# archinetai/audio-diffusion-pytorch

Hardware: NVIDIA H100
Metric: audio-seconds/sec (2ch, 2^18 len) VSampler 50-step (higher is better)
Workload: dtype bf16

## Files before the change

audio_diffusion_pytorch_b200/_build.py:

```python
import os
import subprocess
import sys
from concurrent.futures import ThreadPoolExecutor

PKG_DIR = os.path.dirname(os.path.abspath(__file__))
CSRC = os.path.join(PKG_DIR, "csrc")
LIB_PATH = os.path.join(PKG_DIR, "libadp_b200.so")
SOURCES = ["common.cu", "conv_gemm.cu", "rowwise.cu", "stem.cu", "mid_conv.cu", "attention.cu", "attention_bwd.cu", "backward.cu", "wgrad.cu", "stem_bwd.cu", "frontend.cu", "stft_loss.cu", "verify_f32.cu", "verify_f32_bwd.cu"]
NVCC_FLAGS = [
    "-gencode", "arch=compute_90a,code=sm_90a", "-lineinfo", "-O3", "-std=c++17",
    "-Xcompiler", "-fPIC", "--expt-relaxed-constexpr", "-Xptxas", "-v",
]


def _nvcc() -> str:
    for cand in (os.environ.get("NVCC"), "/usr/local/cuda/bin/nvcc", "nvcc"):
        if cand and (os.path.isabs(cand) and os.path.exists(cand) or not os.path.isabs(cand)):
            return cand
    raise RuntimeError("nvcc not found")


def _sources():
    return [s for s in SOURCES if os.path.exists(os.path.join(CSRC, s))]


def needs_build() -> bool:
    if not os.path.exists(LIB_PATH):
        return True
    lib_m = os.path.getmtime(LIB_PATH)
    deps = [os.path.join(CSRC, f) for f in os.listdir(CSRC)]
    deps.append(os.path.join(os.path.dirname(PKG_DIR), "include", "adp_b200.h"))
    return any(os.path.getmtime(d) > lib_m for d in deps if os.path.exists(d))


def build(force: bool = False, verbose: bool = False) -> str:
    if not force and not needs_build():
        return LIB_PATH
    nvcc = _nvcc()
    objdir = os.path.join(PKG_DIR, "build")
    os.makedirs(objdir, exist_ok=True)

    def compile_one(src: str) -> str:
        obj = os.path.join(objdir, src.replace(".cu", ".o"))
        cmd = [nvcc, *NVCC_FLAGS, "-c", os.path.join(CSRC, src), "-o", obj]
        r = subprocess.run(cmd, capture_output=True, text=True)
        log = os.path.join(objdir, src + ".log")
        with open(log, "w") as fh:
            fh.write(" ".join(cmd) + "\n" + r.stdout + r.stderr)
        if r.returncode != 0:
            raise RuntimeError(f"nvcc failed for {src}:\n{r.stdout}\n{r.stderr}")
        if verbose:
            print(r.stderr, file=sys.stderr)
        return obj

    with ThreadPoolExecutor(max_workers=8) as ex:
        objs = list(ex.map(compile_one, _sources()))
    cmd = [nvcc, "-shared", "-o", LIB_PATH, *objs, "-gencode", "arch=compute_90a,code=sm_90a"]
    r = subprocess.run(cmd, capture_output=True, text=True)
    if r.returncode != 0:
        raise RuntimeError(f"link failed:\n{r.stdout}\n{r.stderr}")
    return LIB_PATH


if __name__ == "__main__":
    print(build(force="--force" in sys.argv, verbose="-v" in sys.argv))
```

audio_diffusion_pytorch_b200/csrc/conv_gemm.cu:

```cuda
#include "common.cuh"
#include "ptx.cuh"

namespace adp {

int g_debug[8] = {0, 0, 0, 0, 0, 0, 0, 0};

constexpr int kMaxStages = 8;
constexpr int kMaxGroups = 8;
constexpr int kSmemPerSM = 228 * 1024;
constexpr int kSmemPerBlock = 227 * 1024;

struct Gemm2Params {
  __nv_bfloat16* out;
  const __nv_bfloat16* residual;
  const float* bias;
  const float* gate;
  double* stats;
  int B, T, tiles_per_batch, c_in, ldo;
  int n_pad, n_valid;
  int ntaps, tap_off0, up_factor;
  int groups, group_size, group_shift;
  int out_fp32, ld_gate;
  int n_tiles_n, total_tiles, tiles_per_cta;
  int a_rows;
  int kc;
  int k_stages;
  int n_stages;
  int a_sub_bytes, w_sub_bytes, stage_bytes, max_taps;
  int early_w;
  const double* gn_stats;
  const float* gn_gamma;
  const float* gn_beta;
  float gn_eps;
  int gn_groups;
};

struct TileInfo {
  int b, t0, n0, phase, ch0, ntaps, min_off;
};

template <int BM>
__device__ __forceinline__ TileInfo tile_info(const Gemm2Params& p, int tile, int BN) {
  TileInfo ti;
  const int m_tile = tile / p.n_tiles_n;
  const int n_tile = tile - m_tile * p.n_tiles_n;
  ti.b = m_tile / p.tiles_per_batch;
  ti.t0 = (m_tile - ti.b * p.tiles_per_batch) * BM;
  ti.n0 = n_tile * BN;
  ti.phase = ti.n0 / p.n_pad;
  ti.ch0 = ti.n0 - ti.phase * p.n_pad;
  if (p.up_factor > 1) {
    if (ti.phase == 0) { ti.ntaps = 2; ti.min_off = -1; }
    else if (ti.phase == p.up_factor - 1) { ti.ntaps = 2; ti.min_off = 0; }
    else { ti.ntaps = 1; ti.min_off = 0; }
  } else {
    ti.ntaps = p.ntaps;
    ti.min_off = p.tap_off0;
  }
  return ti;
}

__device__ __forceinline__ float silu_tanh(float z) {
  float t;
  asm("tanh.approx.f32 %0, %1;" : "=f"(t) : "f"(0.5f * z));
  const float hz = 0.5f * z;
  return fmaf(hz, t, hz);
}

struct WarpStats {
  int cur_g = -1;
  float s = 0.f, q = 0.f;
  template <int NW>
  __device__ __forceinline__ void flush(float (*slots)[NW], int w, int lane) {
    const float ws = warp_sum(s), wq = warp_sum(q);
    if (lane == 0 && cur_g >= 0) { slots[2 * cur_g][w] += ws; slots[2 * cur_g + 1][w] += wq; }
    s = 0.f; q = 0.f;
  }
  template <int NW>
  __device__ __forceinline__ void add(float v, int g, float (*slots)[NW], int w, int lane) {
    if (g != cur_g) { flush(slots, w, lane); cur_g = g; }
    s += v; q += v * v;
  }
};

struct NarrowStats {
  int ch0 = -1;
  float s[4] = {0.f, 0.f, 0.f, 0.f}, q[4] = {0.f, 0.f, 0.f, 0.f};
  __device__ __forceinline__ void add(int k, float v) { s[k] += v; q[k] += v * v; }
  template <int NW>
  __device__ __forceinline__ void flush(float (*slots)[NW], int w, int lane, int shift, int groups) {
    if (ch0 >= 0) {
#pragma unroll
      for (int k = 0; k < 4; ++k) {
        float a = s[k], b = q[k];
#pragma unroll
        for (int o = 4; o < 32; o <<= 1) {
          a += __shfl_xor_sync(0xffffffffu, a, o);
          b += __shfl_xor_sync(0xffffffffu, b, o);
        }
        if (shift == 2) {
          a += __shfl_xor_sync(0xffffffffu, a, 1);
          b += __shfl_xor_sync(0xffffffffu, b, 1);
        }
        const int col = shift == 0 ? ch0 + 2 * lane + k : ch0 + 8 * k + 2 * (lane & 3);
        const int g = col >> shift;
        if (lane < 4 && (shift != 2 || !(lane & 1)) && (shift != 0 || k < 2) && g < groups) {
          slots[2 * g][w] += a;
          slots[2 * g + 1][w] += b;
        }
        s[k] = 0.f; q[k] = 0.f;
      }
    }
    ch0 = -1;
  }
};

template <int BM> constexpr int gemm_threads() { return 2 * BM + 32; }

template <int BM, int BN, int SW, bool XF, bool NARROW>
__global__ void __launch_bounds__(gemm_threads<BM>(), BM == 256 ? 1 : (BN <= 32 ? 3 : (BN <= 64 ? 2 : 1)))
conv_gemm2_kernel(const __grid_constant__ CUtensorMap tmA, const __grid_constant__ CUtensorMap tmW,
                  const Gemm2Params p) {
  static_assert(!NARROW || (BN <= 64 && !XF), "narrow statistics registers: BN <= 64 without XF");
  static_assert(BM == 128 || (BM == 256 && BN == 64 && !XF && !NARROW),
                "256-row tiles: BN = 64, without the A transform or the narrow statistics");
  constexpr int BK = SW / 2;
  constexpr int NACC = BN / 2;
  constexpr int kConsumers = 2 * BM;
  constexpr int kConsumerWarps = BM / 16;
  constexpr uint32_t kWTapBytes = BN * SW;
  extern __shared__ uint8_t smem_raw[];
  __shared__ uint64_t full_bar[kMaxStages], empty_bar[kMaxStages];
  __shared__ float s_part[2 * kMaxGroups][kConsumerWarps];
  __shared__ __align__(16) float s_coef[XF ? 2 * 1024 : 4];

  pdl_launch_dependents();
  const int warp = warp_id_uniform();
  const int lane = threadIdx.x & 31;
  const uint32_t raw = smem_u32(smem_raw);
  uint8_t* ring = smem_raw + ((1024u - (raw & 1023u)) & 1023u);

  const int tile_begin = blockIdx.x * p.tiles_per_cta;
  int tile_end = tile_begin + p.tiles_per_cta;
  if (tile_end > p.total_tiles) tile_end = p.total_tiles;

  if (threadIdx.x < 2 * kMaxGroups * kConsumerWarps) (&s_part[0][0])[threadIdx.x] = 0.f;
  if (warp == kConsumerWarps && lane == 0) {
    for (int s = 0; s < p.n_stages; ++s) { mbar_init(&full_bar[s], 1); mbar_init(&empty_bar[s], kConsumerWarps); }
    fence_mbar_init();
    tma_prefetch_desc(&tmA);
    tma_prefetch_desc(&tmW);
  }
  __syncthreads();
  if (warp == kConsumerWarps) {
    const uint32_t a_bytes = static_cast<uint32_t>(BM / 128) * p.a_rows * SW;
    const int total_it = (tile_end - tile_begin) * p.k_stages;
    int early = 0;
    if (p.early_w) {
      early = total_it < p.n_stages ? total_it : p.n_stages;
      if (elect_one()) {
        int tile = tile_begin, ks = 0;
        for (int it = 0; it < early; ++it) {
          const TileInfo ti = tile_info<BM>(p, tile, BN);
          uint8_t* st = ring + it * p.stage_bytes;
          mbar_arrive_expect_tx(&full_bar[it], static_cast<uint32_t>(p.kc) * (a_bytes + ti.ntaps * kWTapBytes));
          for (int c = 0; c < p.kc; ++c) {
            const int k0 = (ks * p.kc + c) * BK;
            uint8_t* wdst = st + p.kc * p.a_sub_bytes + c * p.max_taps * p.w_sub_bytes;
            for (int tap = 0; tap < ti.ntaps; ++tap)
              tma_load_2d(wdst + tap * p.w_sub_bytes, &tmW, &full_bar[it], tap * p.c_in + k0, ti.n0);
          }
          if (++ks == p.k_stages) { ks = 0; ++tile; }
        }
      }
      __syncwarp();
    }
    pdl_wait();
    int s = 0, it = 0;
    uint32_t ph = 0;
    for (int tile = tile_begin; tile < tile_end; ++tile) {
      const TileInfo ti = tile_info<BM>(p, tile, BN);
      const uint32_t tx = static_cast<uint32_t>(p.kc) * (a_bytes + ti.ntaps * kWTapBytes);
      for (int ks = 0; ks < p.k_stages; ++ks, ++it) {
        const bool armed = it < early;
        if (!armed) mbar_wait(&empty_bar[s], ph ^ 1);
        uint8_t* st = ring + s * p.stage_bytes;
        if (elect_one()) {
          if (!armed) mbar_arrive_expect_tx(&full_bar[s], tx);
          for (int c = 0; c < p.kc; ++c) {
            const int k0 = (ks * p.kc + c) * BK;
            tma_load_3d(st + c * p.a_sub_bytes, &tmA, &full_bar[s], k0, ti.t0 + ti.min_off, ti.b);
            if constexpr (BM == 256)
              tma_load_3d(st + c * p.a_sub_bytes + 128 * SW, &tmA, &full_bar[s], k0, ti.t0 + ti.min_off + 128, ti.b);
            if (armed) continue;
            uint8_t* wdst = st + p.kc * p.a_sub_bytes + c * p.max_taps * p.w_sub_bytes;
            for (int tap = 0; tap < ti.ntaps; ++tap)
              tma_load_2d(wdst + tap * p.w_sub_bytes, &tmW, &full_bar[s], tap * p.c_in + k0, ti.n0);
          }
        }
        __syncwarp();
        if (++s == p.n_stages) { s = 0; ph ^= 1; }
      }
    }
    return;
  }

  pdl_wait();
  const int tid = threadIdx.x;
  const int wg = tid >> 7;
  const int r0 = wg * 64 + (warp & 3) * 16 + (lane >> 2);
  const int cq = 2 * (lane & 3);
  const bool do_stats = p.stats != nullptr;
  const bool narrow = NARROW && p.group_shift >= 0 && p.group_shift < 3;
  WarpStats acc_st;
  NarrowStats nar_st;
  int cur_b = -1, coef_b = -1;

  auto publish_stats = [&](int b_done) {
    acc_st.flush(s_part, warp, lane);
    acc_st.cur_g = -1;
    if (narrow) nar_st.flush(s_part, warp, lane, p.group_shift, p.groups);
    named_bar_sync(1, kConsumers);
    if (tid < 2 * p.groups) {
      float tot = 0.f;
#pragma unroll
      for (int w = 0; w < kConsumerWarps; ++w) { tot += s_part[tid][w]; s_part[tid][w] = 0.f; }
      if (tot != 0.f) atomicAdd(p.stats + static_cast<size_t>(b_done) * 2 * p.groups + tid, static_cast<double>(tot));
    }
    named_bar_sync(1, kConsumers);
  };

  const uint64_t desc0 = gmma_desc_kmajor<SW>(smem_u32(ring));
  const uint32_t stage_u = static_cast<uint32_t>(p.stage_bytes) >> 4;
  const uint32_t a_sub_u = static_cast<uint32_t>(p.a_sub_bytes) >> 4;
  const uint32_t w_sub_u = static_cast<uint32_t>(p.w_sub_bytes) >> 4;
  const uint32_t w_base_u = static_cast<uint32_t>(p.kc) * a_sub_u;
  const uint32_t wg_row_u = static_cast<uint32_t>(wg * 64 * SW) >> 4;
  int s = 0;
  uint32_t ph = 0;
  for (int tile = tile_begin; tile < tile_end; ++tile) {
    const TileInfo ti = tile_info<BM>(p, tile, BN);
    if constexpr (XF) {
      if (ti.b != coef_b) {
        named_bar_sync(1, kConsumers);
        const int gsz = p.c_in / p.gn_groups;
        const double inv_n = 1.0 / (static_cast<double>(gsz) * p.T);
        for (int ch = tid; ch < p.c_in; ch += kConsumers) {
          const int g = ch / gsz;
          const double mean = p.gn_stats[(static_cast<size_t>(ti.b) * p.gn_groups + g) * 2] * inv_n;
          const float var = fmaxf(static_cast<float>(
              p.gn_stats[(static_cast<size_t>(ti.b) * p.gn_groups + g) * 2 + 1] * inv_n - mean * mean), 0.f);
          const float ga = __ldg(p.gn_gamma + ch) * rsqrtf(var + p.gn_eps);
          s_coef[2 * ch] = ga;
          s_coef[2 * ch + 1] = __ldg(p.gn_beta + ch) - static_cast<float>(mean) * ga;
        }
        named_bar_sync(1, kConsumers);
        coef_b = ti.b;
      }
    }
    float acc[NACC];
    uint32_t accumulate = 0;
    int prev_s = -1;
    for (int ks = 0; ks < p.k_stages; ++ks) {
      mbar_wait(&full_bar[s], ph);
      if constexpr (XF) {
        constexpr int CPR = SW / 16;
        constexpr int CPT = CPR / 2 > 0 ? CPR / 2 : 1;
        uint8_t* st = ring + s * p.stage_bytes;
        for (int c = 0; c < p.kc; ++c) {
          uint8_t* sub = st + c * p.a_sub_bytes;
          const float* cf = s_coef + (ks * p.kc + c) * BK * 2;
          for (int rr = tid >> 1; rr < p.a_rows; rr += kConsumers / 2) {
            const int t = ti.t0 + ti.min_off + rr;
            if (t < 0 || t >= p.T) continue;
            const uint32_t row_off = static_cast<uint32_t>(rr) * SW;
            const int swz = (row_off >> 7) & (CPR - 1);
#pragma unroll
            for (int q = 0; q < CPT; ++q) {
              const int pc = (CPR >= 2) ? (tid & 1) * CPT + q : 0;
              if (CPR < 2 && (tid & 1)) continue;
              const int lc = pc ^ swz;
              uint4* ptr = reinterpret_cast<uint4*>(sub + row_off + pc * 16);
              const uint4 u = *ptr;
              const float4* c4 = reinterpret_cast<const float4*>(cf + lc * 16);
              const float4 k0 = c4[0], k1 = c4[1], k2 = c4[2], k3 = c4[3];
              const float2 f0 = unpack_bf16(u.x), f1 = unpack_bf16(u.y);
              const float2 f2 = unpack_bf16(u.z), f3 = unpack_bf16(u.w);
              uint4 o;
              o.x = pack_bf16(silu_tanh(f0.x * k0.x + k0.y), silu_tanh(f0.y * k0.z + k0.w));
              o.y = pack_bf16(silu_tanh(f1.x * k1.x + k1.y), silu_tanh(f1.y * k1.z + k1.w));
              o.z = pack_bf16(silu_tanh(f2.x * k2.x + k2.y), silu_tanh(f2.y * k2.z + k2.w));
              o.w = pack_bf16(silu_tanh(f3.x * k3.x + k3.y), silu_tanh(f3.y * k3.z + k3.w));
              *ptr = o;
            }
          }
        }
        fence_proxy_async_smem();
        named_bar_sync(1, kConsumers);
      }
      wgmma_fence();
      const uint64_t sdesc = desc0 + static_cast<uint64_t>(s * stage_u);
      for (int c = 0; c < p.kc; ++c) {
        const uint64_t adesc = sdesc + c * a_sub_u + wg_row_u;
        const uint64_t wdesc = sdesc + w_base_u + c * p.max_taps * w_sub_u;
        for (int tap = 0; tap < ti.ntaps; ++tap) {
#pragma unroll
          for (int kk = 0; kk < BK / 16; ++kk) {
            Wgmma<BN>::template ss<0, 0>(acc, adesc + ((tap * SW + kk * 32) >> 4),
                                         wdesc + tap * w_sub_u + ((kk * 32) >> 4), accumulate);
            accumulate = 1;
          }
        }
      }
      wgmma_commit();
      wgmma_wait<1>();
      if (prev_s >= 0) {
        __syncwarp();
        if (lane == 0) mbar_arrive(&empty_bar[prev_s]);
      }
      prev_s = s;
      if (++s == p.n_stages) { s = 0; ph ^= 1; }
    }
    wgmma_wait<0>();
    acc_fence(acc);
    __syncwarp();
    if (lane == 0) mbar_arrive(&empty_bar[prev_s]);

    if (do_stats && ti.b != cur_b) {
      if (cur_b >= 0) publish_stats(cur_b);
      cur_b = ti.b;
    }
    if (narrow && ti.ch0 != nar_st.ch0) {
      nar_st.flush(s_part, warp, lane, p.group_shift, p.groups);
      nar_st.ch0 = ti.ch0;
    }
    const int t_lo = ti.t0 + r0, t_hi = t_lo + 8;
    const bool ok_lo = t_lo < p.T, ok_hi = t_hi < p.T;
    const size_t col_off = static_cast<size_t>(ti.phase) * p.n_valid;
    const size_t off_lo = (static_cast<size_t>(ti.b) * p.T + (ok_lo ? t_lo : 0)) * p.ldo + col_off;
    const size_t off_hi = (static_cast<size_t>(ti.b) * p.T + (ok_hi ? t_hi : 0)) * p.ldo + col_off;
    const float* gate_row = p.gate ? p.gate + static_cast<size_t>(ti.b) * p.ld_gate : nullptr;
#pragma unroll
    for (int jb = 0; jb < BN / 8; ++jb) {
      if (ti.ch0 + jb * 8 >= p.n_valid) break;
      const int ch = ti.ch0 + jb * 8 + cq;
      const float2 bb = p.bias ? make_float2(__ldg(p.bias + ch), __ldg(p.bias + ch + 1)) : make_float2(0.f, 0.f);
      const float2 gg = gate_row ? make_float2(__ldg(gate_row + ch), __ldg(gate_row + ch + 1)) : make_float2(1.f, 1.f);
      float v[4];
      v[0] = (acc[4 * jb + 0] + bb.x) * gg.x; v[1] = (acc[4 * jb + 1] + bb.y) * gg.y;
      v[2] = (acc[4 * jb + 2] + bb.x) * gg.x; v[3] = (acc[4 * jb + 3] + bb.y) * gg.y;
      if (p.out_fp32) {
        float* o = reinterpret_cast<float*>(p.out);
        if (ok_lo) *reinterpret_cast<float2*>(o + off_lo + ch) = make_float2(v[0], v[1]);
        if (ok_hi) *reinterpret_cast<float2*>(o + off_hi + ch) = make_float2(v[2], v[3]);
        continue;
      }
      if (p.residual) {
        if (ok_lo) {
          const float2 r = unpack_bf16(__ldg(reinterpret_cast<const unsigned int*>(p.residual + off_lo + ch)));
          v[0] += r.x; v[1] += r.y;
        }
        if (ok_hi) {
          const float2 r = unpack_bf16(__ldg(reinterpret_cast<const unsigned int*>(p.residual + off_hi + ch)));
          v[2] += r.x; v[3] += r.y;
        }
      }
      const uint32_t o_lo = pack_bf16(v[0], v[1]), o_hi = pack_bf16(v[2], v[3]);
      if (ok_lo) *reinterpret_cast<uint32_t*>(p.out + off_lo + ch) = o_lo;
      if (ok_hi) *reinterpret_cast<uint32_t*>(p.out + off_hi + ch) = o_hi;
      if (do_stats) {
        const float2 q_lo = ok_lo ? unpack_bf16(o_lo) : make_float2(0.f, 0.f);
        const float2 q_hi = ok_hi ? unpack_bf16(o_hi) : make_float2(0.f, 0.f);
        if (p.group_shift >= 3) {
          const int g = (ti.ch0 + jb * 8) >> p.group_shift;
          acc_st.add(q_lo.x, g, s_part, warp, lane); acc_st.add(q_lo.y, g, s_part, warp, lane);
          acc_st.add(q_hi.x, g, s_part, warp, lane); acc_st.add(q_hi.y, g, s_part, warp, lane);
        } else if (narrow) {
          if (p.group_shift == 0) {
            nar_st.add(0, q_lo.x); nar_st.add(0, q_hi.x);
            nar_st.add(1, q_lo.y); nar_st.add(1, q_hi.y);
          } else if (jb < 4) {
            nar_st.add(jb, q_lo.x); nar_st.add(jb, q_lo.y);
            nar_st.add(jb, q_hi.x); nar_st.add(jb, q_hi.y);
          }
        } else {
          float cs[2] = {q_lo.x + q_hi.x, q_lo.y + q_hi.y};
          float cs2[2] = {q_lo.x * q_lo.x + q_hi.x * q_hi.x, q_lo.y * q_lo.y + q_hi.y * q_hi.y};
#pragma unroll
          for (int e = 0; e < 2; ++e)
#pragma unroll
            for (int o = 4; o < 32; o <<= 1) {
              cs[e] += __shfl_xor_sync(0xffffffffu, cs[e], o);
              cs2[e] += __shfl_xor_sync(0xffffffffu, cs2[e], o);
            }
#pragma unroll
          for (int i = 0; i < 8; ++i) {
            const float v = __shfl_sync(0xffffffffu, cs[i & 1], i >> 1);
            const float v2 = __shfl_sync(0xffffffffu, cs2[i & 1], i >> 1);
            const int g = (ti.ch0 + jb * 8 + i) / p.group_size;
            if (lane == 0) { s_part[2 * g][warp] += v; s_part[2 * g + 1][warp] += v2; }
          }
        }
      }
    }
  }
  if (do_stats && cur_b >= 0) publish_stats(cur_b);
}

template <int BM, int BN, int SW, bool XF, bool NARROW>
static int launch_gemm2(const adp_conv_gemm_args& a, cudaStream_t stream) {
  constexpr int BK = SW / 2;
  constexpr int kThreads = gemm_threads<BM>();
  auto kernel = conv_gemm2_kernel<BM, BN, SW, XF, NARROW>;
  const int tiles_per_batch = (a.T + BM - 1) / BM;
  const bool up = a.up_factor > 1;
  const int max_taps = up ? 2 : a.ntaps;
  const int span = up ? 1 : a.ntaps - 1;
  const int a_rows = 128 + span;
  const int k_chunks = a.c_in / BK;

  Gemm2Params p;
  p.a_sub_bytes = ((BM + span) * SW + 1023) / 1024 * 1024;
  p.w_sub_bytes = (BN * SW + 1023) / 1024 * 1024;
  p.max_taps = max_taps;
  const int chunk_bytes = p.a_sub_bytes + max_taps * p.w_sub_bytes;

  const int w_iters = k_chunks * max_taps;
  int occ = 1;
  if (BM == 256) occ = 1;
  else if (BN <= 64 && w_iters <= 8) occ = 3;
  else if (BN <= 128 && w_iters <= 12) occ = 2;
  if (XF && occ > (BN <= 64 ? 2 : 1)) occ = BN <= 64 ? 2 : 1;
  if (g_debug[3] > 0) occ = g_debug[3];
  static int static_smem = -1;
  if (static_smem < 0) {
    cudaFuncAttributes fa;
    ADP_CUDA(cudaFuncGetAttributes(&fa, kernel));
    static_smem = static_cast<int>(fa.sharedSizeBytes);
  }
  auto budget_of = [&](int o) {
    int per_cta = kSmemPerSM / o - 1024;
    if (per_cta > kSmemPerBlock) per_cta = kSmemPerBlock;
    return per_cta - static_smem - 1024;
  };
  while (occ > 1 && budget_of(occ) < 2 * chunk_bytes) --occ;
  const int budget = budget_of(occ);
  int kc = 1;
  while (kc * 2 <= 4 && k_chunks % (kc * 2) == 0 && kc * max_taps * (BK / 16) < 8 &&
         2 * (kc * 2) * chunk_bytes <= budget)
    kc *= 2;
  if (g_debug[5] > 0 && k_chunks % g_debug[5] == 0) kc = g_debug[5];
  p.kc = kc;
  p.k_stages = k_chunks / kc;
  p.stage_bytes = kc * chunk_bytes;
  int n_stages = budget / p.stage_bytes;
  if (n_stages > kMaxStages) n_stages = kMaxStages;
  if (n_stages < 2)
    return set_error("adp_conv_gemm: stage of %d bytes does not fit (BN=%d)", p.stage_bytes, BN);
  p.n_stages = n_stages;
  const size_t smem = static_cast<size_t>(n_stages) * p.stage_bytes + 1024;

  CUtensorMap tmA, tmW;
  {
    const uint64_t dims[3] = {(uint64_t)a.c_in, (uint64_t)a.T, (uint64_t)a.B};
    const uint64_t strides[2] = {(uint64_t)a.lda * 2, (uint64_t)a.T * a.lda * 2};
    const uint32_t box[3] = {(uint32_t)BK, (uint32_t)a_rows, 1};
    if (int e = make_tmap_bf16(&tmA, a.a, 3, dims, strides, box, SW)) return e;
  }
  {
    const uint64_t dims[2] = {(uint64_t)a.k_total, (uint64_t)a.phases * a.n_pad};
    const uint64_t strides[1] = {(uint64_t)a.k_total * 2};
    const uint32_t box[2] = {(uint32_t)BK, (uint32_t)BN};
    if (int e = make_tmap_bf16(&tmW, a.w, 2, dims, strides, box, SW)) return e;
  }

  static SmemAttrCache smem_cache;
  ADP_CUDA(ensure_dyn_smem(kernel, smem, smem_cache));
  int occ_hw = 1;
  if (cudaOccupancyMaxActiveBlocksPerMultiprocessor(&occ_hw, kernel, kThreads, smem) != cudaSuccess ||
      occ_hw < 1)
    occ_hw = 1;
  if (occ > occ_hw) occ = occ_hw;

  p.out = static_cast<__nv_bfloat16*>(a.out);
  p.residual = static_cast<const __nv_bfloat16*>(a.residual);
  p.bias = a.bias;
  p.gate = a.gate;
  p.stats = a.stats;
  p.B = a.B;
  p.T = a.T;
  p.tiles_per_batch = tiles_per_batch;
  p.c_in = a.c_in;
  p.ldo = a.ldo;
  p.n_pad = a.n_pad;
  p.n_valid = a.n_valid;
  p.ntaps = a.ntaps;
  p.tap_off0 = a.tap_off[0];
  p.up_factor = a.up_factor;
  p.groups = a.stats ? a.groups : 0;
  p.group_size = a.stats ? a.n_valid / a.groups : 1;
  p.group_shift = -1;
  for (int sft = 0; sft < 16; ++sft)
    if ((1 << sft) == p.group_size) p.group_shift = sft;
  p.out_fp32 = a.out_fp32;
  p.ld_gate = a.ld_gate > 0 ? a.ld_gate : a.n_valid;
  p.n_tiles_n = a.phases * a.n_pad / BN;
  p.total_tiles = a.B * tiles_per_batch * p.n_tiles_n;
  p.a_rows = a_rows;
  p.early_w = g_debug[2];
  p.gn_stats = a.gn_stats;
  p.gn_gamma = a.gn_gamma;
  p.gn_beta = a.gn_beta;
  p.gn_eps = a.gn_eps;
  p.gn_groups = a.gn_groups > 0 ? a.gn_groups : 1;

  const int slots = occ * num_sms();
  int grid = p.total_tiles < slots ? p.total_tiles : slots;
  p.tiles_per_cta = (p.total_tiles + grid - 1) / grid;
  grid = (p.total_tiles + p.tiles_per_cta - 1) / p.tiles_per_cta;
  ADP_CUDA(launch_k(kernel, dim3(grid), dim3(kThreads), smem, stream, tmA, tmW, p));
  ADP_LAUNCH_CHECK();
  return 0;
}

static bool needs_narrow(const adp_conv_gemm_args& a) {
  const int group_size = a.stats ? a.n_valid / a.groups : 0;
  return group_size == 1 || group_size == 2 || group_size == 4 || g_debug[7] != 0;
}

template <int SW>
static int dispatch_bn2(const adp_conv_gemm_args& a, int bn, cudaStream_t s) {
  if (a.gn_stats) {
    switch (bn) {
      case 16: return launch_gemm2<128, 16, SW, true, false>(a, s);
      case 32: return launch_gemm2<128, 32, SW, true, false>(a, s);
      case 64: return launch_gemm2<128, 64, SW, true, false>(a, s);
      case 128: return launch_gemm2<128, 128, SW, true, false>(a, s);
      case 256: return launch_gemm2<128, 256, SW, true, false>(a, s);
    }
  }
  const bool narrow = needs_narrow(a);
  switch (bn) {
    case 16: return narrow ? launch_gemm2<128, 16, SW, false, true>(a, s) : launch_gemm2<128, 16, SW, false, false>(a, s);
    case 32: return narrow ? launch_gemm2<128, 32, SW, false, true>(a, s) : launch_gemm2<128, 32, SW, false, false>(a, s);
    case 64: return narrow ? launch_gemm2<128, 64, SW, false, true>(a, s) : launch_gemm2<128, 64, SW, false, false>(a, s);
    case 128: return launch_gemm2<128, 128, SW, false, false>(a, s);
    case 256: return launch_gemm2<128, 256, SW, false, false>(a, s);
  }
  return set_error("adp_conv_gemm: unsupported N tile %d", bn);
}

static bool has_256_rows(const adp_conv_gemm_args& a) {
  return a.n_pad % 64 == 0 && a.c_in % 64 == 0 && !a.gn_stats && !needs_narrow(a) && a.T >= 256;
}

}

namespace adp { extern int g_mid_threads; }

extern "C" int adp_debug_set(int key, int value) {
  if (key == 8) {
    if (value != 128 && value != 256) return adp::set_error("adp_debug_set: key 8 takes 128 or 256");
    adp::g_mid_threads = value;
    return 0;
  }
  if (key < 0 || key >= 8) return adp::set_error("adp_debug_set: bad key %d", key);
  if (key == 4 && value != 0 && value != 128 && value != 256)
    return adp::set_error("adp_debug_set: key 4 takes 0, 128 or 256");
  adp::g_debug[key] = value;
  if (key == 6) adp::g_pdl = value;
  return 0;
}

extern "C" int adp_conv_gemm(const adp_conv_gemm_args* args, adp_stream_t stream) {
  using namespace adp;
  ADP_CHECK(args != nullptr, "adp_conv_gemm: null args");
  const adp_conv_gemm_args& a = *args;
  ADP_CHECK(a.a && a.w && a.out, "adp_conv_gemm: null a/w/out");
  ADP_CHECK(a.B > 0 && a.T > 0, "adp_conv_gemm: bad B=%d T=%d", a.B, a.T);
  ADP_CHECK(a.c_in >= 16 && a.c_in % 16 == 0, "adp_conv_gemm: c_in=%d must be a multiple of 16",
            a.c_in);
  ADP_CHECK(a.lda % 8 == 0 && a.ldo % 8 == 0 && a.k_total % 8 == 0 && a.lda >= a.c_in,
            "adp_conv_gemm: pitches lda=%d ldo=%d k_total=%d must be multiples of 8", a.lda, a.ldo,
            a.k_total);
  ADP_CHECK(a.n_valid > 0 && a.n_valid % 8 == 0 && a.n_valid <= a.n_pad && a.n_pad % 16 == 0,
            "adp_conv_gemm: n_valid=%d n_pad=%d", a.n_valid, a.n_pad);
  ADP_CHECK(a.phases >= 1, "adp_conv_gemm: phases=%d", a.phases);
  ADP_CHECK(a.ld_gate % 4 == 0, "adp_conv_gemm: ld_gate=%d must be a multiple of 4", a.ld_gate);
  if (a.up_factor > 1) {
    ADP_CHECK(a.phases == a.up_factor, "adp_conv_gemm: phases (%d) != up_factor (%d)", a.phases,
              a.up_factor);
    ADP_CHECK(a.k_total >= 2 * a.c_in, "adp_conv_gemm: upsample weights need 2 tap slots");
  } else {
    ADP_CHECK(a.ntaps >= 1 && a.ntaps <= 3 && a.phases == 1, "adp_conv_gemm: ntaps=%d phases=%d",
              a.ntaps, a.phases);
    ADP_CHECK(a.k_total >= a.ntaps * a.c_in, "adp_conv_gemm: k_total too small");
    for (int i = 1; i < a.ntaps; ++i)
      ADP_CHECK(a.tap_off[i] == a.tap_off[i - 1] + 1,
                "adp_conv_gemm: tap offsets must be consecutive and ascending");
  }
  if (a.out_fp32) {
    ADP_CHECK(!a.residual && !a.stats, "adp_conv_gemm: out_fp32 excludes residual/stats");
  }
  if (a.gn_stats) {
    ADP_CHECK(a.c_in <= 1024, "adp_conv_gemm: fused GroupNorm supports c_in <= 1024");
    ADP_CHECK(a.gn_gamma && a.gn_beta && a.gn_groups > 0 && a.c_in % a.gn_groups == 0 && a.lda == a.c_in,
              "adp_conv_gemm: fused GroupNorm needs gamma/beta, groups | c_in and a dense input");
  }
  if (a.stats) {
    ADP_CHECK(a.groups > 0 && a.groups <= kMaxGroups && a.n_valid % a.groups == 0,
              "adp_conv_gemm: groups=%d n_valid=%d (fused statistics handle <= %d groups)",
              a.groups, a.n_valid, kMaxGroups);
  }
  int bn = a.block_n;
  if (bn == 0) {
    const long m_tiles = (long)a.B * ((a.T + 127) / 128);
    const int k_per_tile = (a.up_factor > 1 ? 2 : a.ntaps) * a.c_in;
    const int widest = !a.gn_stats && k_per_tile <= 1024 ? 64 : 128;
    bn = 16;
    for (int cand = widest; cand >= 16; cand >>= 1) {
      if (a.n_pad % cand) continue;
      const long tiles = m_tiles * (a.phases * a.n_pad / cand);
      if (tiles >= 96 || cand <= 64) { bn = cand; break; }
    }
  }
  bool rows256 = false;
  if (g_debug[4] == 256) {
    ADP_CHECK(has_256_rows(a) && (a.block_n == 0 || a.block_n == 64),
              "adp_conv_gemm: no 256-row tile for block_n=%d c_in=%d T=%d", a.block_n, a.c_in, a.T);
    rows256 = true;
  } else if (a.block_n == 0 && g_debug[4] != 128) {
    rows256 = bn == 128 && has_256_rows(a);
  }
  ADP_CHECK(a.n_pad % bn == 0, "adp_conv_gemm: N tile %d does not divide n_pad %d", bn, a.n_pad);
  cudaStream_t s = as_stream(stream);
  if (rows256) return launch_gemm2<256, 64, 128, false, false>(a, s);
  if (a.c_in % 64 == 0) return dispatch_bn2<128>(a, bn, s);
  if (a.c_in % 32 == 0) return dispatch_bn2<64>(a, bn, s);
  return dispatch_bn2<32>(a, bn, s);
}
```

Before: 173.5.

## Add specialized thin-channel GEMM kernel for small conv and upsample shapes

```diff
diff --git a/audio_diffusion_pytorch_b200/_build.py b/audio_diffusion_pytorch_b200/_build.py
--- a/audio_diffusion_pytorch_b200/_build.py
+++ b/audio_diffusion_pytorch_b200/_build.py
@@ -6,7 +6,7 @@
 PKG_DIR = os.path.dirname(os.path.abspath(__file__))
 CSRC = os.path.join(PKG_DIR, "csrc")
 LIB_PATH = os.path.join(PKG_DIR, "libadp_b200.so")
-SOURCES = ["common.cu", "conv_gemm.cu", "rowwise.cu", "stem.cu", "mid_conv.cu", "attention.cu", "attention_bwd.cu", "backward.cu", "wgrad.cu", "stem_bwd.cu", "frontend.cu", "stft_loss.cu", "verify_f32.cu", "verify_f32_bwd.cu"]
+SOURCES = ["common.cu", "conv_gemm.cu", "rowwise.cu", "stem.cu", "mid_conv.cu", "thin_gemm.cu", "attention.cu", "attention_bwd.cu", "backward.cu", "wgrad.cu", "stem_bwd.cu", "frontend.cu", "stft_loss.cu", "verify_f32.cu", "verify_f32_bwd.cu"]
 NVCC_FLAGS = [
     "-gencode", "arch=compute_90a,code=sm_90a", "-lineinfo", "-O3", "-std=c++17",
     "-Xcompiler", "-fPIC", "--expt-relaxed-constexpr", "-Xptxas", "-v",
diff --git a/audio_diffusion_pytorch_b200/csrc/conv_gemm.cu b/audio_diffusion_pytorch_b200/csrc/conv_gemm.cu
--- a/audio_diffusion_pytorch_b200/csrc/conv_gemm.cu
+++ b/audio_diffusion_pytorch_b200/csrc/conv_gemm.cu
@@ -556,12 +556,22 @@
 
 }
 
-namespace adp { extern int g_mid_threads; }
+namespace adp {
+extern int g_mid_threads;
+bool thin_gemm_fits(const adp_conv_gemm_args& a);
+int thin_gemm(const adp_conv_gemm_args& a, cudaStream_t stream);
+int g_thin_off = 0;
+}
 
 extern "C" int adp_debug_set(int key, int value) {
   if (key == 8) {
     if (value != 128 && value != 256) return adp::set_error("adp_debug_set: key 8 takes 128 or 256");
     adp::g_mid_threads = value;
+    return 0;
+  }
+  if (key == 9) {
+    if (value != 0 && value != 1) return adp::set_error("adp_debug_set: key 9 takes 0 or 1");
+    adp::g_thin_off = value;
     return 0;
   }
   if (key < 0 || key >= 8) return adp::set_error("adp_debug_set: bad key %d", key);
@@ -612,6 +622,7 @@
               "adp_conv_gemm: groups=%d n_valid=%d (fused statistics handle <= %d groups)",
               a.groups, a.n_valid, kMaxGroups);
   }
+  if (!g_thin_off && thin_gemm_fits(a)) return thin_gemm(a, as_stream(stream));
   int bn = a.block_n;
   if (bn == 0) {
     const long m_tiles = (long)a.B * ((a.T + 127) / 128);
diff --git a/audio_diffusion_pytorch_b200/csrc/thin_gemm.cu b/audio_diffusion_pytorch_b200/csrc/thin_gemm.cu
--- /dev/null
+++ b/audio_diffusion_pytorch_b200/csrc/thin_gemm.cu
@@ -0,0 +1,262 @@
+#include "common.cuh"
+#include "ptx.cuh"
+
+namespace adp {
+
+extern int g_debug[8];
+
+__device__ __forceinline__ void cp_async16(uint32_t dst, const void* src, uint32_t src_bytes) {
+  asm volatile("cp.async.cg.shared.global [%0], [%1], 16, %2;" ::"r"(dst), "l"(src), "r"(src_bytes) : "memory");
+}
+__device__ __forceinline__ void cp_async_commit() { asm volatile("cp.async.commit_group;" ::: "memory"); }
+__device__ __forceinline__ void cp_async_wait_1() { asm volatile("cp.async.wait_group 1;" ::: "memory"); }
+
+template <int CIN, int NV, int F, int TB>
+struct ThinCfg {
+  static constexpr int NTH = 2 * TB;
+  static constexpr int HALO = F > 1 ? 1 : 0;
+  static constexpr int AR = TB + 2 * HALO;
+  static constexpr int RS = CIN * 2 + 16;
+  static constexpr int KP = (F > 1 ? 2 : 1) * CIN;
+  static constexpr int WS = KP * 2 + 16;
+  static constexpr int NT = NV / 8;
+  static constexpr int WOUT = F * NV;
+  static constexpr int OS = WOUT + 4;
+  static constexpr int LPR = WOUT / 8;
+  static constexpr int RPP = NTH / LPR;
+  static constexpr int EP = (TB + RPP - 1) / RPP;
+  static constexpr int A_BYTES = AR * RS;
+  static constexpr int O_FLOATS = TB * OS > NTH * 16 ? TB * OS : NTH * 16;
+  static constexpr int W_BYTES = F * NV * WS;
+  static constexpr int SMEM = 2 * A_BYTES + O_FLOATS * 4 + W_BYTES;
+  static_assert(NV % 8 == 0 && CIN % 16 == 0 && TB % 16 == 0 && RPP >= 1, "thin GEMM shape");
+};
+
+template <int CIN, int NV, int F, int TB>
+__global__ void __launch_bounds__(2 * TB, TB == 128 ? 3 : 2) thin_gemm_kernel(const adp_conv_gemm_args a, int early_w) {
+  using Cfg = ThinCfg<CIN, NV, F, TB>;
+  constexpr int NTH = Cfg::NTH, HALO = Cfg::HALO, AR = Cfg::AR, RS = Cfg::RS, KP = Cfg::KP;
+  constexpr int WS = Cfg::WS, NT = Cfg::NT, WOUT = Cfg::WOUT, OS = Cfg::OS, LPR = Cfg::LPR;
+  constexpr int RPP = Cfg::RPP, EP = Cfg::EP;
+  extern __shared__ __align__(128) uint8_t smem[];
+  uint8_t* s_a = smem;
+  float* s_o = reinterpret_cast<float*>(smem + 2 * Cfg::A_BYTES);
+  uint8_t* s_w = smem + 2 * Cfg::A_BYTES + Cfg::O_FLOATS * 4;
+  __shared__ float s_ch[2 * WOUT];
+
+  pdl_launch_dependents();
+  const int b = blockIdx.y;
+  const int tid = threadIdx.x, warp = tid >> 5, lane = tid & 31;
+  const int T = a.T;
+  const int n_tiles = (T + TB - 1) / TB;
+  const __nv_bfloat16* ab = static_cast<const __nv_bfloat16*>(a.a) + static_cast<size_t>(b) * T * a.lda;
+  const size_t orow = static_cast<size_t>(b) * T;
+  const uint32_t a_base = smem_u32(s_a), w_base = smem_u32(s_w);
+
+  auto load_w = [&]() {
+    constexpr int VPR = KP / 8;
+    const __nv_bfloat16* w = static_cast<const __nv_bfloat16*>(a.w);
+    for (int i = tid; i < F * NV * VPR; i += NTH) {
+      const int row = i / VPR, v = i - row * VPR;
+      const int p = row / NV, n = row - p * NV;
+      if (F > 1 && p > 0 && p < F - 1 && v >= CIN / 8) continue;
+      cp_async16(w_base + row * WS + v * 16, w + static_cast<size_t>(p * a.n_pad + n) * a.k_total + v * 8, 16u);
+    }
+  };
+  if (early_w) load_w();
+  pdl_wait();
+  if (!early_w) load_w();
+
+  auto load_a = [&](int tile, int buf) {
+    constexpr int CH = CIN / 8;
+    const int t_first = tile * TB - HALO;
+    for (int i = tid; i < AR * CH; i += NTH) {
+      const int r = i / CH, c = i - r * CH;
+      const int t = t_first + r;
+      const bool ok = t >= 0 && t < T;
+      const __nv_bfloat16* src = ok ? ab + static_cast<size_t>(t) * a.lda + c * 8 : ab;
+      cp_async16(a_base + buf * Cfg::A_BYTES + r * RS + c * 16, src, ok ? 16u : 0u);
+    }
+  };
+
+  int tile = blockIdx.x;
+  if (tile < n_tiles) load_a(tile, 0);
+  cp_async_commit();
+
+  const int el = tid % LPR, row0 = tid / LPR;
+  const bool e_on = row0 < RPP;
+  const int c0 = (el * 8) % NV;
+  float bb[8], gg[8];
+  {
+    const float* gate_row = a.gate ? a.gate + static_cast<size_t>(b) * (a.ld_gate > 0 ? a.ld_gate : a.n_valid) : nullptr;
+#pragma unroll
+    for (int j = 0; j < 8; ++j) {
+      bb[j] = a.bias ? __ldg(a.bias + c0 + j) : 0.f;
+      gg[j] = gate_row ? __ldg(gate_row + c0 + j) : 1.f;
+    }
+  }
+  const bool has_res = a.residual != nullptr;
+  const __nv_bfloat16* res = static_cast<const __nv_bfloat16*>(a.residual);
+  __nv_bfloat16* out = static_cast<__nv_bfloat16*>(a.out);
+  float st_s[8], st_q[8];
+#pragma unroll
+  for (int j = 0; j < 8; ++j) { st_s[j] = 0.f; st_q[j] = 0.f; }
+
+  for (int it = 0; tile < n_tiles; tile += gridDim.x, ++it) {
+    const int buf = it & 1;
+    const int t0 = tile * TB;
+    if (tile + gridDim.x < n_tiles) load_a(tile + gridDim.x, buf ^ 1);
+    cp_async_commit();
+    uint4 rv[EP];
+#pragma unroll
+    for (int i = 0; i < EP; ++i) {
+      const int t = t0 + row0 + i * RPP;
+      rv[i] = make_uint4(0, 0, 0, 0);
+      if (has_res && e_on && row0 + i * RPP < TB && t < T)
+        rv[i] = __ldg(reinterpret_cast<const uint4*>(res + (orow + t) * a.ldo + el * 8));
+    }
+    cp_async_wait_1();
+    __syncthreads();
+
+    const uint32_t ab_s = a_base + buf * Cfg::A_BYTES;
+    const int g = lane >> 2, q = lane & 3;
+#pragma unroll
+    for (int p = 0; p < F; ++p) {
+      const int ntap = (F > 1 && (p == 0 || p == F - 1)) ? 2 : 1;
+      const int off = (F > 1 && p == 0) ? -1 : 0;
+      float acc[NT][4];
+#pragma unroll
+      for (int j = 0; j < NT; ++j) acc[j][0] = acc[j][1] = acc[j][2] = acc[j][3] = 0.f;
+#pragma unroll
+      for (int tap = 0; tap < 2; ++tap) {
+        if (tap >= ntap) break;
+#pragma unroll
+        for (int c16 = 0; c16 < CIN / 16; ++c16) {
+          uint32_t af[4];
+          ldmatrix_x4(ab_s + static_cast<uint32_t>(warp * 16 + (lane & 7) + ((lane >> 3) & 1) * 8 + HALO + off + tap) * RS +
+                      (c16 * 16 + ((lane >> 4) & 1) * 8) * 2, af);
+          const uint32_t wk = w_base + static_cast<uint32_t>(p * NV) * WS + (tap * CIN + c16 * 16) * 2;
+#pragma unroll
+          for (int np = 0; np < NT / 2; ++np) {
+            uint32_t bf[4];
+            ldmatrix_x4(wk + static_cast<uint32_t>(np * 16 + (lane & 7) + ((lane >> 4) & 1) * 8) * WS +
+                        ((lane >> 3) & 1) * 16, bf);
+            mma_16816(acc[2 * np], af, bf[0], bf[1]);
+            mma_16816(acc[2 * np + 1], af, bf[2], bf[3]);
+          }
+          if constexpr (NT % 2 == 1) {
+            uint32_t bf[2];
+            ldmatrix_x2(wk + static_cast<uint32_t>((NT - 1) * 8 + (lane & 7)) * WS + ((lane >> 3) & 1) * 16, bf);
+            mma_16816(acc[NT - 1], af, bf[0], bf[1]);
+          }
+        }
+      }
+      const int r = warp * 16 + g;
+#pragma unroll
+      for (int j = 0; j < NT; ++j) {
+        *reinterpret_cast<float2*>(s_o + r * OS + p * NV + 8 * j + 2 * q) = make_float2(acc[j][0], acc[j][1]);
+        *reinterpret_cast<float2*>(s_o + (r + 8) * OS + p * NV + 8 * j + 2 * q) = make_float2(acc[j][2], acc[j][3]);
+      }
+    }
+    __syncthreads();
+
+#pragma unroll
+    for (int i = 0; i < EP; ++i) {
+      const int rl = row0 + i * RPP;
+      const int t = t0 + rl;
+      if (!e_on || rl >= TB || t >= T) continue;
+      const float4 o0 = *reinterpret_cast<const float4*>(s_o + rl * OS + el * 8);
+      const float4 o1 = *reinterpret_cast<const float4*>(s_o + rl * OS + el * 8 + 4);
+      float y[8] = {o0.x, o0.y, o0.z, o0.w, o1.x, o1.y, o1.z, o1.w};
+#pragma unroll
+      for (int j = 0; j < 8; ++j) y[j] = (y[j] + bb[j]) * gg[j];
+      if (has_res) {
+        const float2 r0 = unpack_bf16(rv[i].x), r1 = unpack_bf16(rv[i].y);
+        const float2 r2 = unpack_bf16(rv[i].z), r3 = unpack_bf16(rv[i].w);
+        y[0] += r0.x; y[1] += r0.y; y[2] += r1.x; y[3] += r1.y;
+        y[4] += r2.x; y[5] += r2.y; y[6] += r3.x; y[7] += r3.y;
+      }
+      uint4 ov;
+      ov.x = pack_bf16(y[0], y[1]); ov.y = pack_bf16(y[2], y[3]);
+      ov.z = pack_bf16(y[4], y[5]); ov.w = pack_bf16(y[6], y[7]);
+      *reinterpret_cast<uint4*>(out + (orow + t) * a.ldo + el * 8) = ov;
+      const float2 q0 = unpack_bf16(ov.x), q1 = unpack_bf16(ov.y);
+      const float2 q2 = unpack_bf16(ov.z), q3 = unpack_bf16(ov.w);
+      const float v[8] = {q0.x, q0.y, q1.x, q1.y, q2.x, q2.y, q3.x, q3.y};
+#pragma unroll
+      for (int j = 0; j < 8; ++j) { st_s[j] += v[j]; st_q[j] = fmaf(v[j], v[j], st_q[j]); }
+    }
+  }
+
+  if (a.stats) {
+    const int gsz = a.n_valid / a.groups;
+    __syncthreads();
+#pragma unroll
+    for (int j = 0; j < 8; ++j) { s_o[tid * 16 + j] = st_s[j]; s_o[tid * 16 + 8 + j] = st_q[j]; }
+    __syncthreads();
+    for (int c = tid; c < 2 * WOUT; c += NTH) {
+      const int ch = c >> 1, which = c & 1;
+      float tot = 0.f;
+      for (int r = 0; r < RPP; ++r) tot += s_o[(r * LPR + ch / 8) * 16 + which * 8 + (ch & 7)];
+      s_ch[c] = tot;
+    }
+    __syncthreads();
+    if (tid < 2 * a.groups) {
+      const int gi = tid >> 1, which = tid & 1;
+      double tot = 0.0;
+      for (int p = 0; p < F; ++p)
+        for (int c = gi * gsz; c < (gi + 1) * gsz; ++c) tot += s_ch[2 * (p * NV + c) + which];
+      if (tot != 0.0) atomicAdd(a.stats + static_cast<size_t>(b) * 2 * a.groups + tid, tot);
+    }
+  }
+}
+
+template <int CIN, int NV, int F, int TB>
+static int launch_thin(const adp_conv_gemm_args& a, cudaStream_t stream) {
+  using Cfg = ThinCfg<CIN, NV, F, TB>;
+  auto kernel = thin_gemm_kernel<CIN, NV, F, TB>;
+  static SmemAttrCache smem_cache;
+  ADP_CUDA(ensure_dyn_smem(kernel, (size_t)Cfg::SMEM, smem_cache));
+  const int gx = one_wave_gx(kernel, Cfg::NTH, (size_t)Cfg::SMEM, a.B, (a.T + TB - 1) / TB);
+  ADP_CUDA(launch_k(kernel, dim3(gx, a.B), dim3(Cfg::NTH), (size_t)Cfg::SMEM, stream, a, g_debug[2]));
+  ADP_LAUNCH_CHECK();
+  return 0;
+}
+
+#define ADP_THIN_SHAPES(X) \
+  X(32, 8, 4, 128)         \
+  X(32, 8, 2, 128)         \
+  X(64, 32, 4, 64)         \
+  X(64, 32, 2, 64)         \
+  X(32, 32, 1, 128)        \
+  X(32, 24, 1, 128)        \
+  X(128, 64, 1, 64)
+
+static int thin_phases(const adp_conv_gemm_args& a) {
+  if (a.up_factor > 1) return a.up_factor;
+  return a.ntaps == 1 && a.tap_off[0] == 0 ? 1 : 0;
+}
+
+static bool aligned16(const void* p) { return (reinterpret_cast<uintptr_t>(p) & 15) == 0; }
+
+bool thin_gemm_fits(const adp_conv_gemm_args& a) {
+  if (a.gn_stats || a.out_fp32 || a.block_n != 0) return false;
+  if (!aligned16(a.a) || !aligned16(a.w) || !aligned16(a.out) || !aligned16(a.residual)) return false;
+  const int f = thin_phases(a);
+#define ADP_THIN_FITS(CIN, NV, F, TB) \
+  if (a.c_in == CIN && a.n_valid == NV && f == F) return true;
+  ADP_THIN_SHAPES(ADP_THIN_FITS)
+#undef ADP_THIN_FITS
+  return false;
+}
+
+int thin_gemm(const adp_conv_gemm_args& a, cudaStream_t stream) {
+  const int f = thin_phases(a);
+#define ADP_THIN_LAUNCH(CIN, NV, F, TB) \
+  if (a.c_in == CIN && a.n_valid == NV && f == F) return launch_thin<CIN, NV, F, TB>(a, stream);
+  ADP_THIN_SHAPES(ADP_THIN_LAUNCH)
+#undef ADP_THIN_LAUNCH
+  return set_error("adp_conv_gemm: no thin GEMM for c_in=%d n_valid=%d phases=%d", a.c_in, a.n_valid, f);
+}
+
+}
```

Measured after the change: 177.2 (median of 6 runs). +2.2%, better.
